# esa-prl/planning-motion_planning

Measured on AMD Instinct MI355X. Metric: Eikonal Gcells/s + ms-to-path, 4k² & 16k² costmap at 1/2/4/8 GPU, higher is better.
Workload: dtype f64; 1 GPU; C2: 4096x4096 DEM-derived cost raster, single goal, FIM on 1 MI355X; H=4096, W=4096, split=1x1, tile=64, parallelism=single-gpu

## Files before the change

planning-motion_planning_amd/csrc/fim2d.hip:

```cpp
#include "fim_engine.hpp"

namespace eik {

template <typename R>
__device__ __forceinline__ R stage_cost(R c) {
    if constexpr (sizeof(R) == 8 && EIK_CHAIN) return (c >= R(0) && c < 0x1p-500) ? R(0x1p-500) : c;
    else return c;
}


#ifndef EIK_ACT_STEP
#define EIK_ACT_STEP 0
#endif
constexpr int kActStep = EIK_ACT_STEP;



#ifndef EIK_ECOL_F64
#define EIK_ECOL_F64 1
#endif
#ifndef EIK_ECOL_F32
#define EIK_ECOL_F32 0
#endif
template <typename R>
constexpr bool kEcol = sizeof(R) == 8 ? EIK_ECOL_F64 : EIK_ECOL_F32;

#ifndef EIK_FRESH_SKIP
#define EIK_FRESH_SKIP 1
#endif
constexpr bool kFreshSkip = EIK_FRESH_SKIP;

template <typename R>
struct alignas(2 * sizeof(R)) Cell {
    R t, c;
};

#ifndef EIK_SWZ
#define EIK_SWZ 0
#endif
__device__ __forceinline__ constexpr int cell_swz(int col) { return EIK_SWZ ? (col >> 4) & 1 : 0; }
template <typename R>
__device__ __forceinline__ R& cell_t(Cell<R>* Ts, int idx, int col) {
    return reinterpret_cast<R*>(Ts + idx)[cell_swz(col)];
}
template <typename R>
__device__ __forceinline__ R& cell_c(Cell<R>* Ts, int idx, int col) {
    return reinterpret_cast<R*>(Ts + idx)[1 - cell_swz(col)];
}
template <typename R>
__device__ __forceinline__ Cell<R> make_cell(R t, R c, int col) {
    return cell_swz(col) ? Cell<R>{c, t} : Cell<R>{t, c};
}


#ifndef EIK_SWEEP_UNROLL
#define EIK_SWEEP_UNROLL 4
#endif
#ifndef EIK_SWEEP_UNROLL_F32
#define EIK_SWEEP_UNROLL_F32 8
#endif
template <typename R, int DX, int DY, bool TRACK, bool REF = false, class Hook>
__device__ __forceinline__ bool sweep_quadrant(Cell<R>* __restrict__ Ts, int lane, R keep, Hook&& hook) {
    constexpr int S = (int)sizeof(Cell<R>);
    constexpr int kRow = kLds * S;
    constexpr int D = kAhead;
    static_assert((2 * kTile) % D == 0, "pipeline depth must divide the step count");
    char* const base = reinterpret_cast<char*>(Ts);
    const int col = (DX > 0 ? lane : kTile - 1 - lane) + 1;
    constexpr int RB = (int)sizeof(R);
    const int colT = col * S + cell_swz(col) * RB;
    const int dC = (1 - 2 * cell_swz(col)) * RB;
    const int dU = (col - DX) * S + cell_swz(col - DX) * RB - colT;
    const int lo_b = -(D - 1) * kRow + colT, hi_b = (kLds - 1) * kRow + colT;
    int raw = DY > 0 ? (1 - lane) * kRow + colT : (kTile - (D - 1) + lane) * kRow + colT;
    auto off = [](int u) { return (DY > 0 ? u : D - 1 - u) * kRow; };
    auto clampb = [&](int x) {
        int r;
        asm("v_med3_i32 %0, %1, %2, %3" : "=v"(r) : "v"(x), "v"(lo_b), "v"(hi_b));
        return r;
    };
    bool changed = false;
    R cur = *reinterpret_cast<const R*>(base + (DY > 0 ? 0 : kLds - 1) * kRow + colT);
    R q_old[D], q_upx[D], q_c[D];
    int gb = clampb(raw);
    raw += DY * D * kRow;
    auto fetch = [&](int u) {
        const int o = gb + off(u);
#if EIK_SWZ
        q_old[u] = *reinterpret_cast<const R*>(base + o);
        q_c[u] = *reinterpret_cast<const R*>(base + o + dC);
#else
        const Cell<R> v = *reinterpret_cast<const Cell<R>*>(base + o);
        q_old[u] = v.t;
        q_c[u] = v.c;
#endif
        q_upx[u] = *reinterpret_cast<const R*>(base + o + dU);
    };
#pragma unroll
    for (int u = 0; u < D; ++u) fetch(u);
    constexpr int kUnroll = sizeof(R) == 8 ? EIK_SWEEP_UNROLL : EIK_SWEEP_UNROLL_F32;
#pragma unroll kUnroll
    for (int s = 0; s < 2 * kTile; s += D) {
        hook(s);
        const int gcur = gb;
        gb = clampb(raw);
        raw += DY * D * kRow;
#pragma unroll
        for (int u = 0; u < D; ++u) {
            const R c2x2 = R(2) * (q_c[u] * q_c[u]);
            R w;
            if constexpr (sizeof(R) == 8) {
                if constexpr (REF) w = eik_ref(wave_shr1(cur, q_upx[u]), cur, q_c[u]);
                else w = godunov2_chain(wave_shr1(cur, q_upx[u]), cur, q_c[u], c2x2);
                lds_min(reinterpret_cast<R*>(base + gcur + off(u)), w);
                if constexpr (TRACK) changed |= w < q_old[u] * keep;
                cur = fmin_nn(w, q_old[u]);
            } else {
                w = godunov2_chain(umin(wave_shr1_umin_id(cur), q_upx[u]), cur, q_c[u], c2x2);
                lds_min(reinterpret_cast<R*>(base + gcur + off(u)), w);
                if constexpr (TRACK) changed |= w < q_old[u] * keep;
                cur = umin(w, q_old[u]);
            }
            fetch(u);
            __builtin_amdgcn_sched_barrier(0);
        }
    }
    return changed;
}
template <typename R, int DX, int DY, bool TRACK, bool REF = false>
__device__ __forceinline__ bool sweep_quadrant(Cell<R>* __restrict__ Ts, int lane, R keep) {
    return sweep_quadrant<R, DX, DY, TRACK, REF>(Ts, lane, keep, [](int) {});
}

template <typename R>
struct TileLds {
    Cell<R> Tc[(kLds + 2 * kGuard) * kLds];
    unsigned round, flags;
    unsigned flags_acc;
    unsigned pend;
    unsigned key[5];
    int defer, tile, last;
    unsigned dirs;
    unsigned fresh;
};

template <typename R, bool COH, bool CAP = false, bool REF = false>
__device__ __forceinline__ void process_tile(const Fim2dArgs& a, int tile, TileLds<R>& L, R keep) {
    constexpr R INF = Real<R>::inf();
    Cell<R>* const Ts = L.Tc + kGuard * kLds;
    const int tid = threadIdx.x, lane = tid & 63, wave = tid >> 6;
    const int map = tile / a.tiles_per_map;
    const int rem = tile - map * a.tiles_per_map;
    const int ty = rem / a.ntx, tx = rem - (rem / a.ntx) * a.ntx;
    const R* __restrict__ cost = static_cast<const R*>(a.cost) + (int64_t)map * a.H * a.W;
    const TMem<R, COH> T(static_cast<R*>(a.T) + (int64_t)map * a.H * a.W, a.H * a.W);
    const TMem<R, COH> E(static_cast<R*>(a.ecol), (int64_t)a.capacity * 2 * kTile);
    auto eidx = [&](int t, int side, int row) { return ((int64_t)t * 2 + side) * kTile + row; };
    const int64_t y0 = (int64_t)ty * kTile, x0 = (int64_t)tx * kTile;
    const bool full = (y0 + kTile <= a.H) && (x0 + kTile <= a.W) && ((a.W & 3) == 0);
    const R capv = CAP ? (R)a.tcap[map] : INF;

    EIK_PROBE(0);
    if (tid == 0) {
        L.round = 0;
        L.flags = 0;
        L.flags_acc = 0;
        L.pend = 0;
    }
    if (tid < 5) L.key[tid] = 0x7f800000u;
    const int64_t sy = y0 + kTile < a.H ? y0 + kTile : a.H;
    const int64_t sx = x0 + kTile < a.W ? x0 + kTile : a.W;
    struct Halo {
        int h, hcol;
        int64_t hy, hx, idx;
        bool in;
    };
    auto halo_of = [&](int k) {
        Halo q;
        if (k == 0)      { q.hcol = lane + 1;            q.h = 0 * kLds + q.hcol; }
        else if (k == 1) { q.hcol = lane + 1;            q.h = (int)(sy - y0 + 1) * kLds + q.hcol; }
        else if (k == 2) { q.hcol = 0;                   q.h = (lane + 1) * kLds + q.hcol; }
        else             { q.hcol = (int)(sx - x0 + 1);  q.h = (lane + 1) * kLds + q.hcol; }
        q.hy = k == 0 ? y0 - 1 : k == 1 ? sy : y0 + lane;
        q.hx = k == 0 || k == 1 ? x0 + lane : k == 2 ? x0 - 1 : sx;
        q.in = q.hy >= 0 && q.hy < a.H && q.hx >= 0 && q.hx < a.W;
        q.idx = q.in ? q.hy * a.W + q.hx : 0;
        if (kEcol<R> && k >= 2 && q.in) q.idx = eidx(k == 2 ? tile - 1 : tile + 1, k == 2 ? 1 : 0, lane);
        return q;
    };
    auto load_halo_of = [&](const Halo& q, int k) {
        R v = kEcol<R> && k >= 2 ? E.ld(q.idx) : T.ld(q.idx);
        if (!q.in) v = load_T<R, COH>(a, T, q.hy, q.hx);
        return v;
    };
    const Halo hw = halo_of(wave);
    const int h = hw.h, hcol = hw.hcol;
    auto load_halo = [&]() { return load_halo_of(hw, wave); };
    R told[16];
    const int cx = (tid & 15) * 4;
    auto store_tile = [&](const R (&cr)[16], R hv) {
#pragma unroll
        for (int k = 0; k < 4; ++k) {
            const int ry = (tid >> 4) + 16 * k;
#pragma unroll
            for (int e = 0; e < 4; ++e)
                Ts[(ry + 1) * kLds + cx + e + 1] = make_cell<R>(told[4 * k + e], stage_cost(cr[4 * k + e]), cx + e + 1);
        }
        Ts[h] = make_cell<R>(hv, INF, hcol);
    };
    if (full && COH && kFreshSkip && __builtin_amdgcn_readfirstlane(L.fresh)) {
        R cr[16];
#pragma unroll
        for (int k = 0; k < 4; ++k) {
            const int64_t gy = y0 + (tid >> 4) + 16 * k;
            if constexpr (sizeof(R) == 4) {
                const float4 c4 = *reinterpret_cast<const float4*>(&cost[gy * a.W + x0 + cx]);
                cr[4 * k] = c4.x; cr[4 * k + 1] = c4.y; cr[4 * k + 2] = c4.z; cr[4 * k + 3] = c4.w;
            } else {
                const double2 c0 = *reinterpret_cast<const double2*>(&cost[gy * a.W + x0 + cx]);
                const double2 c1 = *reinterpret_cast<const double2*>(&cost[gy * a.W + x0 + cx + 2]);
                cr[4 * k] = c0.x; cr[4 * k + 1] = c0.y; cr[4 * k + 2] = c1.x; cr[4 * k + 3] = c1.y;
            }
#pragma unroll
            for (int e = 0; e < 4; ++e) told[4 * k + e] = INF;
        }
        store_tile(cr, load_halo());
        if (tid == 0) atomicAdd(a.visits + 2, 1ull);
    } else if (full) {
        R cr[16];
#pragma unroll
        for (int k = 0; k < 4; ++k) {
            const int64_t gy = y0 + (tid >> 4) + 16 * k;
            R tv[4];
            T.ld4(gy * a.W + x0 + cx, tv);
            if constexpr (sizeof(R) == 4) {
                const float4 c4 = *reinterpret_cast<const float4*>(&cost[gy * a.W + x0 + cx]);
                cr[4 * k] = c4.x; cr[4 * k + 1] = c4.y; cr[4 * k + 2] = c4.z; cr[4 * k + 3] = c4.w;
            } else {
                const double2 c0 = *reinterpret_cast<const double2*>(&cost[gy * a.W + x0 + cx]);
                const double2 c1 = *reinterpret_cast<const double2*>(&cost[gy * a.W + x0 + cx + 2]);
                cr[4 * k] = c0.x; cr[4 * k + 1] = c0.y; cr[4 * k + 2] = c1.x; cr[4 * k + 3] = c1.y;
            }
#pragma unroll
            for (int e = 0; e < 4; ++e) told[4 * k + e] = tv[e];
        }
        store_tile(cr, load_halo());
    } else {
        R cr[16];
#pragma unroll
        for (int k = 0; k < 4; ++k) {
            const int64_t gy = y0 + (tid >> 4) + 16 * k;
#pragma unroll
            for (int e = 0; e < 4; ++e) {
                const int64_t gx = x0 + cx + e;
                const bool in = gy < a.H && gx < a.W;
                told[4 * k + e] = load_T<R, COH>(a, T, gy, gx);
                cr[4 * k + e] = in ? cost[gy * a.W + gx] : INF;
            }
        }
        store_tile(cr, load_halo());
        if (tid < kLds) {
            if (sy - y0 < kTile) Ts[(kLds - 1) * kLds + tid] = Cell<R>{INF, INF};
            if (sx - x0 < kTile) Ts[tid * kLds + (kLds - 1)] = Cell<R>{INF, INF};
        }
    }
    if (lane < 4) cell_c(Ts, (lane >> 1) * (kLds - 1) * kLds + (lane & 1) * (kLds - 1), (lane & 1) * (kLds - 1)) = INF;
    __syncthreads();
    EIK_PROBE(1);
    if constexpr (CAP) asm volatile("" ::"v"(capv));

    unsigned dirs = L.dirs;
    int act_tile = -1;
    unsigned act_old = 0u, act_kold = 0x7f800000u;
    float act_k = 0.f;
    auto act_complete = [&]() {
        if (act_tile >= 0) qpush_complete(a, act_tile, act_old, act_k, act_kold);
        act_tile = -1;
    };
    for (int pass = 0;; ++pass) {
        auto hook = [&](int st) {
            if (EIK_ACT_SPLIT && wave == 0 && st == kActStep) act_complete();
        };
        const bool sweep = (dirs >> wave) & 1u;
        bool last_changed = false;
        if (a.max_rounds == 1) {
            if (sweep) {
                if (wave == 0)      sweep_quadrant<R, +1, +1, false, REF>(Ts, lane, keep, hook);
                else if (wave == 1) sweep_quadrant<R, -1, +1, false, REF>(Ts, lane, keep, hook);
                else if (wave == 2) sweep_quadrant<R, +1, -1, false, REF>(Ts, lane, keep, hook);
                else                sweep_quadrant<R, -1, -1, false, REF>(Ts, lane, keep, hook);
            } else {
                for (int st = 0; st < 2 * kTile; st += kAhead) hook(st);
            }
            __syncthreads();
        } else {
            for (int round = 0;; ++round) {
                bool ch = false;
                if (sweep) {
                    if (wave == 0)      ch = sweep_quadrant<R, +1, +1, true, REF>(Ts, lane, keep);
                    else if (wave == 1) ch = sweep_quadrant<R, -1, +1, true, REF>(Ts, lane, keep);
                    else if (wave == 2) ch = sweep_quadrant<R, +1, -1, true, REF>(Ts, lane, keep);
                    else                ch = sweep_quadrant<R, -1, -1, true, REF>(Ts, lane, keep);
                }
                if (__any(ch) && lane == 0) atomicOr(&L.round, 1u << (round & 31));
                __syncthreads();
                last_changed = (L.round >> (round & 31)) & 1u;
                if (!last_changed || round + 1 >= a.max_rounds) break;
            }
        }

        EIK_PROBE(2);
        unsigned pend_old = 0;
        R nv[16];
#pragma unroll
        for (int k = 0; k < 4; ++k) {
            const int ry = (tid >> 4) + 16 * k;
#pragma unroll
            for (int e = 0; e < 4; ++e) nv[4 * k + e] = cell_t(Ts, (ry + 1) * kLds + cx + e + 1, cx + e + 1);
        }
        unsigned chg = 0;
#pragma unroll
        for (int k = 0; k < 4; ++k) {
            const int ry = (tid >> 4) + 16 * k;
            const int64_t gy = y0 + ry;
            bool any = false;
#pragma unroll
            for (int e = 0; e < 4; ++e) {
                const int i = 4 * k + e;
                any |= nv[i] < told[i];
                const bool in = full || (gy < a.H && x0 + cx + e < a.W);
                chg |= (nv[i] < told[i] * keep && in) ? 1u << i : 0u;
            }
            if (any) {
                if (full) {
                    const R v[4] = {nv[4 * k], nv[4 * k + 1], nv[4 * k + 2], nv[4 * k + 3]};
                    T.st4(gy * a.W + x0 + cx, v);
                } else {
#pragma unroll
                    for (int e = 0; e < 4; ++e) {
                        const int64_t gx = x0 + cx + e;
                        if (gy < a.H && gx < a.W && nv[4 * k + e] < told[4 * k + e]) T.st(gy * a.W + gx, nv[4 * k + e]);
                    }
                }
                if (kEcol<R> && cx == 0 && nv[4 * k] < told[4 * k]) E.st(eidx(tile, 0, ry), nv[4 * k]);
                if (kEcol<R> && cx == kTile - 4 && nv[4 * k + 3] < told[4 * k + 3]) E.st(eidx(tile, 1, ry), nv[4 * k + 3]);
            }
        }
        if (COH && (a.sched & 1) && tid == 0)
            pend_old = atomicAnd(&a.qstate[tile + (int)__builtin_amdgcn_mbcnt_lo(0u, 0u)], kBusy | kVisited);
        __builtin_amdgcn_sched_barrier(0);
        if (COH) {
#pragma unroll
            for (int i = 0; i < 16; ++i) told[i] = nv[i];
        }
        const bool keys = a.delta < INF || a.bctl;
        unsigned fl = chg ? 128u : 0u;
        R kmin_self = INF, kmin[4] = {INF, INF, INF, INF};
        if (keys) {
#pragma unroll
            for (int i = 0; i < 16; ++i) kmin_self = umin(kmin_self, (chg >> i) & 1u ? nv[i] : INF);
        }
        auto edge = [&](int q, int i0, int di, int h0, int dh, int hc) {
            R hv[4];
#pragma unroll
            for (int j = 0; j < 4; ++j) hv[j] = cell_t(Ts, h0 + dh * j, hc < 0 ? cx + j + 1 : hc);
#pragma unroll
            for (int j = 0; j < 4; ++j) {
                const int i = i0 + di * j;
                const bool act = !CAP || nv[i] <= capv;
                const bool hit = ((chg >> i) & 1u) && act && nv[i] < hv[j];
                fl |= hit ? 1u << q : 0u;
                kmin[q] = umin(kmin[q], hit ? nv[i] : INF);
            }
        };
        const int ly0 = (tid >> 4) + 1;
        if ((tid >> 4) == 0) edge(0, 0, 1, cx + 1, 1, -1);
        if ((tid >> 4) == 15) edge(1, 12, 1, (kLds - 1) * kLds + cx + 1, 1, -1);
        if ((tid & 15) == 0) edge(2, 0, 4, ly0 * kLds, 16 * kLds, 0);
        if ((tid & 15) == 15) edge(3, 3, 4, ly0 * kLds + kLds - 1, 16 * kLds, kLds - 1);
        if (!full) {
#pragma unroll
            for (int k = 0; k < 4; ++k) {
                const int ry = (tid >> 4) + 16 * k;
                if (y0 + ry == a.H - 1 && ry != kTile - 1 && ((chg >> (4 * k)) & 0xFu)) fl |= 32u;
            }
#pragma unroll
            for (int e = 0; e < 4; ++e)
                if (x0 + cx + e == a.W - 1 && cx + e != kTile - 1 && (chg & (0x1111u << e))) fl |= 64u;
        }
        const unsigned wfl = wave_reduce_idem(fl, [](unsigned x, unsigned y) { return x | y; });
        if (wfl && lane == 0) atomicOr(&L.flags, wfl);
        if (keys) {
            const R km[5] = {kmin_self, kmin[0], kmin[1], kmin[2], kmin[3]};
#pragma unroll
            for (int q = 0; q < 5; ++q) {
                const unsigned wk = wave_reduce_idem(__float_as_uint((float)km[q]), [](unsigned x, unsigned y) { return min(x, y); });
                if (wk < 0x7f800000u && lane == 0) atomicMin(&L.key[q], wk);
            }
        }
        if (tid == 0) L.last = a.max_rounds == 1 ? -1 : (int)last_changed;
        if constexpr (COH) {
            __builtin_amdgcn_s_waitcnt(0x0F70);
            asm volatile("s_waitcnt vmcnt(0)" ::: "memory");
        }
        if (COH && (a.sched & 1) && tid == 0) L.pend = pend_old;
        __syncthreads();
        EIK_PROBE(7);
        if (COH) {
            const unsigned f = L.flags;
            const unsigned pend = L.pend & (kPending | kFromN | kFromS | kFromW | kFromE);
            const bool self = (f & 128u) != 0u;
            if ((!self && !pend) || pass + 1 >= a.max_passes || a.max_rounds != 1) break;
            const R hv = load_halo();
            if (tid == 64) charge_inplace_pass(a);
            const bool defer = (a.sched & 2) && pass > 0;
            if constexpr (EIK_ACT_SPLIT)
                act_tile = activate_neighbours_issue(a, tile, defer ? 0u : f, act_old, L.key, act_k,
                                                     act_kold);
            else
                activate_neighbours(a, tile, defer ? 0u : f, L.key, 0, 0u);
            if (defer && tid == 0) L.flags_acc |= f & 0x6fu;
            dirs = self ? 0xFu : sweep_dirs(pend);
            cell_t(Ts, h, hcol) = hv;
            __syncthreads();
            if (tid == 0) {
                L.flags = 0;
                L.pend = 0;
            }
        } else {
            break;
        }
    }
    act_complete();
    EIK_PROBE(3);
}

template <typename R>
__device__ __forceinline__ void activate_after(const Fim2dArgs& a, int tile, const TileLds<R>& L, int list,
                                               unsigned stamp) {
    const unsigned f = L.flags;
    activate_neighbours(a, tile, f | L.flags_acc, L.key, list, stamp);
    if (threadIdx.x == 0) {
        const bool self = L.last < 0 ? (f & 128u) != 0u : L.last != 0;
        if (a.mode == kModePersistent) {
            const unsigned p = L.pend & (kFromN | kFromS | kFromW | kFromE);
            if (self || (L.pend & kPending)) {
                if (self && a.bctl) atomicMin(&a.key[tile], 0u);
                atomicOr(&a.qstate[tile], kPending | (self ? kSelf : p));
            }
        } else if (self) {
            enqueue(a, tile, list, stamp, __uint_as_float(L.key[0]));
        }
    }
}

template <typename R>
__device__ __forceinline__ void init_guard_rows(TileLds<R>& L) {
    const int tid = threadIdx.x;
    for (int i = tid; i < kGuard * kLds; i += kThreads) {
        L.Tc[i] = Cell<R>{Real<R>::inf(), Real<R>::inf()};
        L.Tc[(kLds + kGuard) * kLds + i] = Cell<R>{Real<R>::inf(), Real<R>::inf()};
    }
}

template <typename R>
__global__ __launch_bounds__(kThreads) void fim2d_sweep_kernel(Fim2dArgs a) {
    constexpr R INF = Real<R>::inf();
    __shared__ TileLds<R> L;
    const int tid = threadIdx.x;
    init_guard_rows(L);
    const int cur = a.iter % 3, nxt = (a.iter + 1) % 3, rst = (a.iter + 2) % 3;
    const int cnt = a.counts[cur];
    if (blockIdx.x == 0 && tid == 0) {
        a.counts[rst] = 0;
        a.minkey[rst] = 0x7f800000u;
    }
    const unsigned stamp = a.iter + 2;
    const float thr = __uint_as_float(a.minkey[cur]) + a.delta;
    const R keep = (R)a.keep;
    if (tid == 0) L.dirs = 0xFu;

    for (int it = blockIdx.x; it < cnt; it += gridDim.x) {
        const int tile = a.lists[(int64_t)cur * a.capacity + it];
        if (a.delta < INF) {
            if (tid == 0) {
                const float k = __uint_as_float(atomicOr(&a.key[tile], 0u));
                L.defer = k > thr;
                if (k > thr) enqueue(a, tile, nxt, stamp, k);
                else atomicExch(&a.key[tile], 0x7f800000u);
            }
            __syncthreads();
            const bool defer = L.defer;
            __syncthreads();
            if (defer) continue;
        }
        process_tile<R, false>(a, tile, L, keep);
        activate_after(a, tile, L, nxt, stamp);
        if (tid == 0 && a.visits) atomicAdd(a.visits, 1ull);
        __syncthreads();
    }
}

template <typename R>
__device__ __forceinline__ void merge_strip_cells(const Fim2dArgs& a, int side, const R* rv, R* g, int64_t i,
                                                  int64_t len, unsigned* count) {
    R v = Real<R>::inf();
    bool drop = false;
    if (i < len) {
        v = ld_system(rv + i);
        drop = v < ld_agent(g + i);
        if (drop) st_scoped(g + i, v, __HIP_MEMORY_SCOPE_AGENT);
    }
    const unsigned long long m = __ballot(drop);
    if (!m) return;
    __builtin_amdgcn_fence(__ATOMIC_RELEASE, "agent");
    unsigned k = drop ? __float_as_uint((float)v) : 0x7f800000u;
#pragma unroll
    for (int d = 32; d > 0; d >>= 1) k = min(k, (unsigned)__shfl_xor((int)k, d));
    if ((threadIdx.x & 63) == (unsigned)__builtin_ctzll(m)) {
        if (count) atomicAdd(count, (unsigned)__popcll(m));
        int ty, tx;
        if (side < 2) {
            tx = (int)(i / kTile);
            ty = side == 0 ? 0 : a.nty - 1;
        } else {
            ty = (int)(i / kTile);
            tx = side == 2 ? 0 : a.ntx - 1;
        }
        activate(a, ty * a.ntx + tx, a.iter % 3, a.iter + 1, __uint_as_float(k), kFromN << side);
    }
}

template <typename R>
__device__ __forceinline__ void live_agent(const Fim2dArgs& a, unsigned* sh) {
    const int tid = threadIdx.x;
    auto pack = [&](unsigned par, bool skip_busy) {
        const R* T = static_cast<const R*>(a.T);
        R* tg[4];
        for (int k = 0; k < 4; ++k) tg[k] = static_cast<R*>(a.live->send[par][k]);
        auto idle = [&](int64_t ty, int64_t tx) {
            return !skip_busy ||
                   (__hip_atomic_load(&a.qstate[ty * a.ntx + tx], __ATOMIC_RELAXED, __HIP_MEMORY_SCOPE_AGENT) &
                    (kPending | kBusy)) == 0u;
        };
        for (int64_t i = tid; i < a.W; i += blockDim.x) {
            if (tg[0] && idle(0, i / kTile)) st_scoped(tg[0] + i, ld_agent(T + i), __HIP_MEMORY_SCOPE_SYSTEM);
            if (tg[1] && idle(a.nty - 1, i / kTile))
                st_scoped(tg[1] + i, ld_agent(T + (a.H - 1) * a.W + i), __HIP_MEMORY_SCOPE_SYSTEM);
        }
        for (int64_t i = tid; i < a.H; i += blockDim.x) {
            if (tg[2] && idle(i / kTile, 0)) st_scoped(tg[2] + i, ld_agent(T + i * a.W), __HIP_MEMORY_SCOPE_SYSTEM);
            if (tg[3] && idle(i / kTile, a.ntx - 1))
                st_scoped(tg[3] + i, ld_agent(T + i * a.W + a.W - 1), __HIP_MEMORY_SCOPE_SYSTEM);
        }
    };
    auto merge = [&](unsigned par, unsigned* count) {
        for (int side = 0; side < 4; ++side) {
            const R* rv = static_cast<const R*>(a.live->recv[par][side]);
            R* g = static_cast<R*>(const_cast<void*>(a.ghost[side]));
            if (!rv || !g) continue;
            const int64_t len = side < 2 ? a.W : a.H;
            for (int64_t i0 = 0; i0 < len; i0 += blockDim.x) merge_strip_cells<R>(a, side, rv, g, i0 + tid, len, count);
        }
    };
    live_agent_loop(a, sh, pack, merge);
}

template <typename R, int WPS, bool REF>
constexpr int kPersistWaves = WPS > 1 ? WPS : sizeof(R) == 4 ? 3 : REF ? 1 : 2;
template <typename R, int WPS, bool CAP = false, bool REF = false>
__global__ __launch_bounds__(kThreads, (kPersistWaves<R, WPS, REF>)) void fim2d_persist_kernel(Fim2dArgs a) {
    __shared__ TileLds<R> L;
    if (a.live && blockIdx.x == 0) {
        __shared__ unsigned sh[4];
        live_agent<R>(a, sh);
        return;
    }
    init_guard_rows(L);
    EIK_KSTART();
    const R keep = (R)a.keep;
    int tile = -1;
    unsigned nvis = 0;
    for (;;) {
        if (threadIdx.x < 64) {
            if (tile >= 0) {
                EIK_PROBE(4);
                activate_after(a, tile, L, 0, 0u);
                asm volatile("s_waitcnt vmcnt(0)" ::: "memory");
                if (threadIdx.x == 0) {
                    qfinish(a, tile);
                    if (++nvis == 64u) {
                        charge_visits(a, 64ull);
                        nvis = 0;
                    }
                }
            }
            EIK_PROBE(5);
        } else if (threadIdx.x < 128 && (a.bctl || threadIdx.x == 64)) {
            unsigned trig = 0;
            const int t = a.bctl ? qgrab_prio(a, trig) : qgrab(a, trig);
            if (threadIdx.x == 64) {
                L.tile = t;
                L.dirs = sweep_dirs(trig);
                L.fresh = !(trig & kVisited);
                if (t >= 0) EIK_VISIT(t, trig, L.dirs);
            }
        }
        __syncthreads();
        EIK_PROBE(6);
        tile = __builtin_amdgcn_readfirstlane(L.tile);
        if (tile < 0) break;
        process_tile<R, true, CAP, REF>(a, tile, L, keep);
    }
    if (threadIdx.x == 0 && nvis) atomicAdd(a.visits, (unsigned long long)nvis);
}
template <typename R>
__global__ void fim2d_init_kernel(R* __restrict__ T, int64_t n, unsigned* __restrict__ mark, int64_t ntiles,
                                  unsigned* __restrict__ key, unsigned* __restrict__ minkey, unsigned* __restrict__ qstate,
                                  unsigned* __restrict__ qslot, int64_t nslots, unsigned* __restrict__ counts,
                                  unsigned* __restrict__ qctl, unsigned* __restrict__ visits, unsigned* __restrict__ edge,
                                  R* __restrict__ ecol) {
    const int64_t stride = (int64_t)gridDim.x * blockDim.x;
    if (blockIdx.x == 0 && threadIdx.x < kQueueCtlBytes / 4) {
        const int t = threadIdx.x;
        if (qctl) qctl[t] = 0u;
        if (t < 4) {
            if (counts) counts[t] = 0u;
            if (edge) edge[t] = 0u;
        }
        if (t < 22 && visits) visits[t] = 0u;
    }
    for (int64_t i = (int64_t)blockIdx.x * blockDim.x + threadIdx.x; i < n; i += stride) T[i] = Real<R>::inf();
    if (ecol)
        for (int64_t i = (int64_t)blockIdx.x * blockDim.x + threadIdx.x; i < ntiles * 2 * kTile; i += stride)
            ecol[i] = Real<R>::inf();
    for (int64_t i = (int64_t)blockIdx.x * blockDim.x + threadIdx.x; i < ntiles; i += stride) {
        mark[i] = 0;
        key[i] = 0x7f800000u;
        if (qstate) qstate[i] = 0;
    }
    for (int64_t i = (int64_t)blockIdx.x * blockDim.x + threadIdx.x; i < nslots; i += stride) qslot[i] = 0;
    if (blockIdx.x == 0 && threadIdx.x < 3) minkey[threadIdx.x] = threadIdx.x == 0 ? 0u : 0x7f800000u;
}

template <typename R>
__global__ void fim2d_seed_kernel(Fim2dArgs a, const int64_t* __restrict__ goals, int nmaps) {
    const int m = blockIdx.x * blockDim.x + threadIdx.x;
    if (m == 0) {
        a.counts[1] = 0;
        a.counts[2] = 0;
    }
    if (m >= nmaps) return;
    const int64_t gx = goals[2 * m], gy = goals[2 * m + 1];
    if (gx < 0 || gy < 0 || gx >= a.W || gy >= a.H) return;
    static_cast<R*>(a.T)[(int64_t)m * a.H * a.W + gy * a.W + gx] = R(0);
    const int tile = m * a.tiles_per_map + (int)(gy / kTile) * a.ntx + (int)(gx / kTile);
    if (kEcol<R> && a.ecol && (gx % kTile == 0 || gx % kTile == kTile - 1))
        static_cast<R*>(a.ecol)[((int64_t)tile * 2 + (gx % kTile == 0 ? 0 : 1)) * kTile + gy % kTile] = R(0);
    if (a.mode == kModePersistent) {
        qpush(a, tile, kSelf | kVisited);
        return;
    }
    a.mark[tile] = 1;
    a.key[tile] = 0u;
    const int pos = atomicAdd(&a.counts[0], 1);
    a.lists[pos] = tile;
}

template <typename R>
__global__ __launch_bounds__(256) void prio_delta_kernel(const R* __restrict__ cost, int64_t n, float mult,
                                                          float* __restrict__ out) {
    __shared__ double ssum[4];
    __shared__ int scnt[4];
    double sum = 0.0;
    int cnt = 0;
    for (int i = threadIdx.x; i < 4096; i += 256) {
        const unsigned long long hsh = (unsigned long long)(i + 1) * 0x9E3779B97F4A7C15ull;
        const double c = (double)cost[(int64_t)((hsh >> 11) % (unsigned long long)n)];
        if (c > 0.0 && c < Real<double>::inf()) {
            sum += log(c);
            ++cnt;
        }
    }
    for (int d = 32; d > 0; d >>= 1) {
        sum += __shfl_down(sum, d);
        cnt += __shfl_down(cnt, d);
    }
    if ((threadIdx.x & 63) == 0) {
        ssum[threadIdx.x >> 6] = sum;
        scnt[threadIdx.x >> 6] = cnt;
    }
    __syncthreads();
    if (threadIdx.x == 0) {
        const double s = ssum[0] + ssum[1] + ssum[2] + ssum[3];
        const int c = scnt[0] + scnt[1] + scnt[2] + scnt[3];
        const double g = c ? exp(s / c) : 1.0;
        *out = (float)(mult * 64.0 * g > 1e-30 ? mult * 64.0 * g : 1e-30);
    }
}

hipError_t fim2d_prio_delta(const void* cost, bool f64, int64_t n, float mult, float* out, hipStream_t st) {
    if (f64)
        hipLaunchKernelGGL(prio_delta_kernel<double>, dim3(1), dim3(256), 0, st, static_cast<const double*>(cost), n,
                           mult, out);
    else
        hipLaunchKernelGGL(prio_delta_kernel<float>, dim3(1), dim3(256), 0, st, static_cast<const float*>(cost), n,
                           mult, out);
    return hipGetLastError();
}

__global__ void fim2d_qrewind_kernel(Fim2dArgs a) {
    if (a.bctl) {
        const int64_t stride = (int64_t)gridDim.x * blockDim.x;
        for (int64_t i = (int64_t)blockIdx.x * blockDim.x + threadIdx.x; i <= (int64_t)a.qmask; i += stride) {
            const unsigned v = a.qslot[i];
            if (v == 0u) continue;
            const unsigned tag = v >> kBandTagShift;
            if (tag) atomicAnd(&a.bmem[(v & kSlotTileMask) - 1u], ~(1ull << (tag - 1u)));
            a.qslot[i] = 0u;
        }
    }
    if (blockIdx.x == 0 && threadIdx.x == 0) *a.qhead = *a.qtail;
}
static void launch_qrewind(const Fim2dArgs& a, hipStream_t st) {
    const int grid = a.bctl ? (int)std::min<int64_t>(256, ((int64_t)a.qmask + 256) / 256) : 1;
    hipLaunchKernelGGL(fim2d_qrewind_kernel, dim3(grid), dim3(a.bctl ? 256 : 1), 0, st, a);
}

template <typename R>
__global__ __launch_bounds__(256) void fim2d_merge_ghost_kernel(Fim2dArgs a, int side, const R* __restrict__ recv,
                                                                int64_t len) {
    R* g = static_cast<R*>(const_cast<void*>(a.ghost[side]));
    merge_strip_cells<R>(a, side, recv, g, (int64_t)blockIdx.x * blockDim.x + threadIdx.x, len, nullptr);
}

template <typename R>
__global__ void fim2d_pack_edges_kernel(Fim2dArgs a, R* __restrict__ n, R* __restrict__ s, R* __restrict__ w,
                                        R* __restrict__ e) {
    const int64_t i = (int64_t)blockIdx.x * blockDim.x + threadIdx.x;
    const R* T = static_cast<const R*>(a.T);
    if (i < a.W) {
        if (n) st_scoped(n + i, ld_agent(T + i), __HIP_MEMORY_SCOPE_SYSTEM);
        if (s) st_scoped(s + i, ld_agent(T + (a.H - 1) * a.W + i), __HIP_MEMORY_SCOPE_SYSTEM);
    }
    if (i < a.H) {
        if (w) st_scoped(w + i, ld_agent(T + i * a.W), __HIP_MEMORY_SCOPE_SYSTEM);
        if (e) st_scoped(e + i, ld_agent(T + i * a.W + a.W - 1), __HIP_MEMORY_SCOPE_SYSTEM);
    }
}

hipError_t fim2d_sweep(const Fim2dArgs& a, bool f64, int grid, hipStream_t st) {
    if (f64)
        hipLaunchKernelGGL(fim2d_sweep_kernel<double>, dim3(grid), dim3(kThreads), 0, st, a);
    else
        hipLaunchKernelGGL(fim2d_sweep_kernel<float>, dim3(grid), dim3(kThreads), 0, st, a);
    return hipGetLastError();
}

int fim2d_persist_resident(bool f64, int cus, bool wide) {
    int per_cu = 0;
    const hipError_t e =
        f64    ? hipOccupancyMaxActiveBlocksPerMultiprocessor(&per_cu, fim2d_persist_kernel<double, 1>, kThreads, 0)
        : wide ? hipOccupancyMaxActiveBlocksPerMultiprocessor(&per_cu, fim2d_persist_kernel<float, 4>, kThreads, 0)
               : hipOccupancyMaxActiveBlocksPerMultiprocessor(&per_cu, fim2d_persist_kernel<float, 1>, kThreads, 0);
    if (e != hipSuccess || per_cu < 1) per_cu = 1;
    return per_cu * cus;
}

hipError_t fim2d_persist(const Fim2dArgs& a, bool f64, int grid, hipStream_t st, bool wide, bool rewind) {
    if (f64 && a.ref_arith && a.tcap)
        hipLaunchKernelGGL((fim2d_persist_kernel<double, 1, true, true>), dim3(grid), dim3(kThreads), 0, st, a);
    else if (f64 && a.ref_arith)
        hipLaunchKernelGGL((fim2d_persist_kernel<double, 1, false, true>), dim3(grid), dim3(kThreads), 0, st, a);
    else if (f64 && a.tcap)
        hipLaunchKernelGGL((fim2d_persist_kernel<double, 1, true>), dim3(grid), dim3(kThreads), 0, st, a);
    else if (f64)
        hipLaunchKernelGGL((fim2d_persist_kernel<double, 1>), dim3(grid), dim3(kThreads), 0, st, a);
    else if (wide)
        hipLaunchKernelGGL((fim2d_persist_kernel<float, 4>), dim3(grid), dim3(kThreads), 0, st, a);
    else
        hipLaunchKernelGGL((fim2d_persist_kernel<float, 1>), dim3(grid), dim3(kThreads), 0, st, a);
    if (rewind) launch_qrewind(a, st);
    return hipGetLastError();
}

hipError_t fim2d_qrewind(const Fim2dArgs& a, hipStream_t st) {
    launch_qrewind(a, st);
    return hipGetLastError();
}

hipError_t fim2d_init(const Fim2dArgs& a, bool f64, int nmaps, const int64_t* d_goals, unsigned* edge, hipStream_t st) {
    static_assert(kQueueCtlBytes / 4 <= 256, "the init kernel's block 0 clears the queue words");
    const int64_t n = (int64_t)nmaps * a.H * a.W;
    const int64_t ntiles = (int64_t)nmaps * a.tiles_per_map;
    const int grid = (int)std::min<int64_t>(4096, (n + 255) / 256);
    const int64_t nslots = a.qslot ? (int64_t)a.qmask + 1 : 0;
    unsigned* const counts = reinterpret_cast<unsigned*>(a.counts);
    unsigned* const qctl = reinterpret_cast<unsigned*>(a.qhead);
    unsigned* const visits = reinterpret_cast<unsigned*>(a.visits);
    if (f64) {
        hipLaunchKernelGGL(fim2d_init_kernel<double>, dim3(grid), dim3(256), 0, st, static_cast<double*>(a.T), n,
                           a.mark, ntiles, a.key, a.minkey, a.qstate, a.qslot, nslots, counts, qctl, visits, edge,
                           kEcol<double> ? static_cast<double*>(a.ecol) : nullptr);
        hipLaunchKernelGGL(fim2d_seed_kernel<double>, dim3((nmaps + 255) / 256), dim3(256), 0, st, a, d_goals, nmaps);
    } else {
        hipLaunchKernelGGL(fim2d_init_kernel<float>, dim3(grid), dim3(256), 0, st, static_cast<float*>(a.T), n,
                           a.mark, ntiles, a.key, a.minkey, a.qstate, a.qslot, nslots, counts, qctl, visits, edge,
                           kEcol<float> ? static_cast<float*>(a.ecol) : nullptr);
        hipLaunchKernelGGL(fim2d_seed_kernel<float>, dim3((nmaps + 255) / 256), dim3(256), 0, st, a, d_goals, nmaps);
    }
    return hipGetLastError();
}

hipError_t fim2d_merge_ghost(const Fim2dArgs& a, bool f64, int side, const void* recv, int64_t len, hipStream_t st) {
    const int grid = (int)((len + 255) / 256);
    if (f64)
        hipLaunchKernelGGL(fim2d_merge_ghost_kernel<double>, dim3(grid), dim3(256), 0, st, a, side,
                           static_cast<const double*>(recv), len);
    else
        hipLaunchKernelGGL(fim2d_merge_ghost_kernel<float>, dim3(grid), dim3(256), 0, st, a, side,
                           static_cast<const float*>(recv), len);
    return hipGetLastError();
}

hipError_t fim2d_pack_edges(const Fim2dArgs& a, bool f64, void* n, void* s, void* w, void* e, hipStream_t st) {
    const int64_t len = a.H > a.W ? a.H : a.W;
    const int grid = (int)((len + 255) / 256);
    if (f64)
        hipLaunchKernelGGL(fim2d_pack_edges_kernel<double>, dim3(grid), dim3(256), 0, st, a, (double*)n, (double*)s,
                           (double*)w, (double*)e);
    else
        hipLaunchKernelGGL(fim2d_pack_edges_kernel<float>, dim3(grid), dim3(256), 0, st, a, (float*)n, (float*)s,
                           (float*)w, (float*)e);
    return hipGetLastError();
}

}
```

Before: 8.599 Gcells/s.

## Precompute halo source pointers, pin tile geometry in SGPRs, clamp edge-tile loads

Tile geometry is passed in a struct pinned to scalar registers, and the wave index is made uniform. Halo loads on full tiles now take a per-wave base pointer and stride chosen branchlessly, including ghost buffers, instead of recomputing per-lane bounds logic. Partial-edge f64 tiles use clamped unconditional loads followed by masking, and store predicates reuse a precomputed in-bounds mask. The seed kernel also activates neighbouring tiles when the goal sits on a tile edge, which changes scheduling slightly and adds complexity and some risk in the ghost and edge handling.

```diff
diff --git a/planning-motion_planning_amd/csrc/fim2d.hip b/planning-motion_planning_amd/csrc/fim2d.hip
--- a/planning-motion_planning_amd/csrc/fim2d.hip
+++ b/planning-motion_planning_amd/csrc/fim2d.hip
@@ -29,6 +29,9 @@
 #define EIK_FRESH_SKIP 1
 #endif
 constexpr bool kFreshSkip = EIK_FRESH_SKIP;
+
+template <typename R>
+constexpr bool kCutWide = sizeof(R) == 8;
 
 template <typename R>
 struct alignas(2 * sizeof(R)) Cell {
@@ -144,20 +147,25 @@
     unsigned fresh;
 };
 
+struct TileGeom {
+    int64_t H, W;
+    int ntx, tiles_per_map, max_passes;
+};
 template <typename R, bool COH, bool CAP = false, bool REF = false>
-__device__ __forceinline__ void process_tile(const Fim2dArgs& a, int tile, TileLds<R>& L, R keep) {
+__device__ __forceinline__ void process_tile(const Fim2dArgs& a, const TileGeom& g, int tile, TileLds<R>& L, R keep) {
     constexpr R INF = Real<R>::inf();
     Cell<R>* const Ts = L.Tc + kGuard * kLds;
-    const int tid = threadIdx.x, lane = tid & 63, wave = tid >> 6;
-    const int map = tile / a.tiles_per_map;
-    const int rem = tile - map * a.tiles_per_map;
-    const int ty = rem / a.ntx, tx = rem - (rem / a.ntx) * a.ntx;
-    const R* __restrict__ cost = static_cast<const R*>(a.cost) + (int64_t)map * a.H * a.W;
-    const TMem<R, COH> T(static_cast<R*>(a.T) + (int64_t)map * a.H * a.W, a.H * a.W);
+    const int tid = threadIdx.x, lane = tid & 63;
+    const int wave = __builtin_amdgcn_readfirstlane(tid >> 6);
+    const int map = tile / g.tiles_per_map;
+    const int rem = tile - map * g.tiles_per_map;
+    const int ty = rem / g.ntx, tx = rem - (rem / g.ntx) * g.ntx;
+    const R* __restrict__ cost = static_cast<const R*>(a.cost) + (int64_t)map * g.H * g.W;
+    const TMem<R, COH> T(static_cast<R*>(a.T) + (int64_t)map * g.H * g.W, g.H * g.W);
     const TMem<R, COH> E(static_cast<R*>(a.ecol), (int64_t)a.capacity * 2 * kTile);
     auto eidx = [&](int t, int side, int row) { return ((int64_t)t * 2 + side) * kTile + row; };
     const int64_t y0 = (int64_t)ty * kTile, x0 = (int64_t)tx * kTile;
-    const bool full = (y0 + kTile <= a.H) && (x0 + kTile <= a.W) && ((a.W & 3) == 0);
+    const bool full = (y0 + kTile <= g.H) && (x0 + kTile <= g.W) && ((g.W & 3) == 0);
     const R capv = CAP ? (R)a.tcap[map] : INF;
 
     EIK_PROBE(0);
@@ -168,8 +176,8 @@
         L.pend = 0;
     }
     if (tid < 5) L.key[tid] = 0x7f800000u;
-    const int64_t sy = y0 + kTile < a.H ? y0 + kTile : a.H;
-    const int64_t sx = x0 + kTile < a.W ? x0 + kTile : a.W;
+    const int64_t sy = y0 + kTile < g.H ? y0 + kTile : g.H;
+    const int64_t sx = x0 + kTile < g.W ? x0 + kTile : g.W;
     struct Halo {
         int h, hcol;
         int64_t hy, hx, idx;
@@ -183,22 +191,55 @@
         else             { q.hcol = (int)(sx - x0 + 1);  q.h = (lane + 1) * kLds + q.hcol; }
         q.hy = k == 0 ? y0 - 1 : k == 1 ? sy : y0 + lane;
         q.hx = k == 0 || k == 1 ? x0 + lane : k == 2 ? x0 - 1 : sx;
-        q.in = q.hy >= 0 && q.hy < a.H && q.hx >= 0 && q.hx < a.W;
-        q.idx = q.in ? q.hy * a.W + q.hx : 0;
+        q.in = q.hy >= 0 && q.hy < g.H && q.hx >= 0 && q.hx < g.W;
+        q.idx = q.in ? q.hy * g.W + q.hx : 0;
         if (kEcol<R> && k >= 2 && q.in) q.idx = eidx(k == 2 ? tile - 1 : tile + 1, k == 2 ? 1 : 0, lane);
         return q;
     };
-    auto load_halo_of = [&](const Halo& q, int k) {
+    const bool ghosts = a.ghost[0] || a.ghost[1] || a.ghost[2] || a.ghost[3];
+    auto load_halo_of = [&](int k) {
+        const Halo q = halo_of(k);
         R v = kEcol<R> && k >= 2 ? E.ld(q.idx) : T.ld(q.idx);
-        if (!q.in) v = load_T<R, COH>(a, T, q.hy, q.hx);
+        if (ghosts) {
+            if (!q.in) v = load_T<R, COH>(a, T, q.hy, q.hx);
+        } else {
+            v = q.in ? v : INF;
+        }
         return v;
     };
-    const Halo hw = halo_of(wave);
-    const int h = hw.h, hcol = hw.hcol;
-    auto load_halo = [&]() { return load_halo_of(hw, wave); };
+    const int hcol = wave < 2 ? lane + 1 : wave == 2 ? 0 : (int)(sx - x0 + 1);
+    const int h = (wave == 0 ? 0 : wave == 1 ? (int)(sy - y0 + 1) : lane + 1) * kLds + hcol;
+    TMem<R, COH> HM = T;
+    int hidx = 0;
+    bool hsrc = true;
+    auto halo_source = [&]() {
+        if constexpr (COH) {
+            const bool row = wave < 2;
+            const bool in = wave == 0 ? y0 > 0 : wave == 1 ? sy < g.H : wave == 2 ? x0 > 0 : sx < g.W;
+            auto gbits = [&](int k) { return reinterpret_cast<uintptr_t>(a.ghost[k]) & (uintptr_t)0 - (uintptr_t)(wave == k); };
+            R* const gs = reinterpret_cast<R*>(gbits(0) | gbits(1) | gbits(2) | gbits(3));
+            R* const Tm = static_cast<R*>(a.T) + (int64_t)map * g.H * g.W;
+            const bool ecol = kEcol<R> && !row;
+            R* const base = !in ? gs : ecol ? static_cast<R*>(a.ecol) : Tm;
+            const int64_t n = !in ? (gs ? (row ? g.W : g.H) : 0) : ecol ? (int64_t)a.capacity * 2 * kTile : (int64_t)g.H * g.W;
+            const int64_t first = !in    ? (row ? x0 : y0)
+                                  : row  ? (wave == 0 ? y0 - 1 : sy) * g.W + x0
+                                  : ecol ? eidx(wave == 2 ? tile - 1 : tile + 1, wave == 2 ? 1 : 0, 0)
+                                         : y0 * g.W + (wave == 2 ? x0 - 1 : sx);
+            const int64_t stride = in && !row && !ecol ? g.W : 1;
+            HM = TMem<R, COH>(base, n);
+            hidx = (int)(first + lane * stride);
+            hsrc = in || gs;
+        }
+    };
+    auto halo_issue_full = [&]() -> R {
+        if constexpr (COH) return HM.ld(hidx);
+        else return load_halo_of(wave);
+    };
     R told[16];
+    unsigned inm = 0xFFFFu;
     const int cx = (tid & 15) * 4;
-    auto store_tile = [&](const R (&cr)[16], R hv) {
+    auto store_tile = [&](const R (&cr)[16], R hv, bool src) {
 #pragma unroll
         for (int k = 0; k < 4; ++k) {
             const int ry = (tid >> 4) + 16 * k;
@@ -206,7 +247,8 @@
             for (int e = 0; e < 4; ++e)
                 Ts[(ry + 1) * kLds + cx + e + 1] = make_cell<R>(told[4 * k + e], stage_cost(cr[4 * k + e]), cx + e + 1);
         }
-        Ts[h] = make_cell<R>(hv, INF, hcol);
+        if (src) Ts[h] = make_cell<R>(hv, INF, hcol);
+        else Ts[h] = make_cell<R>(INF, INF, hcol);
     };
     if (full && COH && kFreshSkip && __builtin_amdgcn_readfirstlane(L.fresh)) {
         R cr[16];
@@ -214,17 +256,20 @@
         for (int k = 0; k < 4; ++k) {
             const int64_t gy = y0 + (tid >> 4) + 16 * k;
             if constexpr (sizeof(R) == 4) {
-                const float4 c4 = *reinterpret_cast<const float4*>(&cost[gy * a.W + x0 + cx]);
+                const float4 c4 = *reinterpret_cast<const float4*>(&cost[gy * g.W + x0 + cx]);
                 cr[4 * k] = c4.x; cr[4 * k + 1] = c4.y; cr[4 * k + 2] = c4.z; cr[4 * k + 3] = c4.w;
             } else {
-                const double2 c0 = *reinterpret_cast<const double2*>(&cost[gy * a.W + x0 + cx]);
-                const double2 c1 = *reinterpret_cast<const double2*>(&cost[gy * a.W + x0 + cx + 2]);
+                const double2 c0 = *reinterpret_cast<const double2*>(&cost[gy * g.W + x0 + cx]);
+                const double2 c1 = *reinterpret_cast<const double2*>(&cost[gy * g.W + x0 + cx + 2]);
                 cr[4 * k] = c0.x; cr[4 * k + 1] = c0.y; cr[4 * k + 2] = c1.x; cr[4 * k + 3] = c1.y;
             }
 #pragma unroll
             for (int e = 0; e < 4; ++e) told[4 * k + e] = INF;
         }
-        store_tile(cr, load_halo());
+        halo_source();
+        const R hraw = halo_issue_full();
+        __builtin_amdgcn_sched_barrier(0);
+        store_tile(cr, hraw, !COH || hsrc);
         if (tid == 0) atomicAdd(a.visits + 2, 1ull);
     } else if (full) {
         R cr[16];
@@ -232,33 +277,63 @@
         for (int k = 0; k < 4; ++k) {
             const int64_t gy = y0 + (tid >> 4) + 16 * k;
             R tv[4];
-            T.ld4(gy * a.W + x0 + cx, tv);
+            T.ld4(gy * g.W + x0 + cx, tv);
             if constexpr (sizeof(R) == 4) {
-                const float4 c4 = *reinterpret_cast<const float4*>(&cost[gy * a.W + x0 + cx]);
+                const float4 c4 = *reinterpret_cast<const float4*>(&cost[gy * g.W + x0 + cx]);
                 cr[4 * k] = c4.x; cr[4 * k + 1] = c4.y; cr[4 * k + 2] = c4.z; cr[4 * k + 3] = c4.w;
             } else {
-                const double2 c0 = *reinterpret_cast<const double2*>(&cost[gy * a.W + x0 + cx]);
-                const double2 c1 = *reinterpret_cast<const double2*>(&cost[gy * a.W + x0 + cx + 2]);
+                const double2 c0 = *reinterpret_cast<const double2*>(&cost[gy * g.W + x0 + cx]);
+                const double2 c1 = *reinterpret_cast<const double2*>(&cost[gy * g.W + x0 + cx + 2]);
                 cr[4 * k] = c0.x; cr[4 * k + 1] = c0.y; cr[4 * k + 2] = c1.x; cr[4 * k + 3] = c1.y;
             }
 #pragma unroll
             for (int e = 0; e < 4; ++e) told[4 * k + e] = tv[e];
         }
-        store_tile(cr, load_halo());
+        halo_source();
+        const R hraw = halo_issue_full();
+        __builtin_amdgcn_sched_barrier(0);
+        store_tile(cr, hraw, !COH || hsrc);
     } else {
         R cr[16];
+        inm = 0u;
+        const int rmax = (int)(g.H - 1 - y0), cmax = (int)(g.W - 1 - x0);
+        const int64_t org = y0 * g.W + x0;
 #pragma unroll
         for (int k = 0; k < 4; ++k) {
-            const int64_t gy = y0 + (tid >> 4) + 16 * k;
+            const int ry = (tid >> 4) + 16 * k;
+            const int row = (ry < rmax ? ry : rmax) * (int)g.W;
 #pragma unroll
             for (int e = 0; e < 4; ++e) {
-                const int64_t gx = x0 + cx + e;
-                const bool in = gy < a.H && gx < a.W;
-                told[4 * k + e] = load_T<R, COH>(a, T, gy, gx);
-                cr[4 * k + e] = in ? cost[gy * a.W + gx] : INF;
-            }
-        }
-        store_tile(cr, load_halo());
+                const bool in = ry <= rmax && cx + e <= cmax;
+                const int64_t idx = org + (row + (cx + e < cmax ? cx + e : cmax));
+                inm |= in ? 1u << (4 * k + e) : 0u;
+                if constexpr (kCutWide<R>) {
+                    told[4 * k + e] = T.ld(idx);
+                    cr[4 * k + e] = cost[idx];
+                } else {
+                    told[4 * k + e] = load_T<R, COH>(a, T, y0 + ry, x0 + cx + e);
+                    cr[4 * k + e] = in ? cost[(y0 + ry) * g.W + x0 + cx + e] : INF;
+                }
+            }
+        }
+        const R hv = load_halo_of(wave);
+        if constexpr (kCutWide<R>) {
+            if (ghosts) {
+#pragma unroll
+                for (int k = 0; k < 4; ++k) {
+                    const int64_t gy = y0 + (tid >> 4) + 16 * k;
+#pragma unroll
+                    for (int e = 0; e < 4; ++e)
+                        if (!((inm >> (4 * k + e)) & 1u)) told[4 * k + e] = load_T<R, COH>(a, T, gy, x0 + cx + e);
+                }
+            } else {
+#pragma unroll
+                for (int i = 0; i < 16; ++i) told[i] = (inm >> i) & 1u ? told[i] : INF;
+            }
+#pragma unroll
+            for (int i = 0; i < 16; ++i) cr[i] = (inm >> i) & 1u ? cr[i] : INF;
+        }
+        store_tile(cr, hv, true);
         if (tid < kLds) {
             if (sy - y0 < kTile) Ts[(kLds - 1) * kLds + tid] = Cell<R>{INF, INF};
             if (sx - x0 < kTile) Ts[tid * kLds + (kLds - 1)] = Cell<R>{INF, INF};
@@ -319,6 +394,8 @@
             for (int e = 0; e < 4; ++e) nv[4 * k + e] = cell_t(Ts, (ry + 1) * kLds + cx + e + 1, cx + e + 1);
         }
         unsigned chg = 0;
+        unsigned inp = inm;
+        asm volatile("" : "+v"(inp));
 #pragma unroll
         for (int k = 0; k < 4; ++k) {
             const int ry = (tid >> 4) + 16 * k;
@@ -328,24 +405,24 @@
             for (int e = 0; e < 4; ++e) {
                 const int i = 4 * k + e;
                 any |= nv[i] < told[i];
-                const bool in = full || (gy < a.H && x0 + cx + e < a.W);
-                chg |= (nv[i] < told[i] * keep && in) ? 1u << i : 0u;
+                chg |= nv[i] < told[i] * keep ? 1u << i : 0u;
             }
             if (any) {
                 if (full) {
                     const R v[4] = {nv[4 * k], nv[4 * k + 1], nv[4 * k + 2], nv[4 * k + 3]};
-                    T.st4(gy * a.W + x0 + cx, v);
+                    T.st4(gy * g.W + x0 + cx, v);
                 } else {
 #pragma unroll
                     for (int e = 0; e < 4; ++e) {
                         const int64_t gx = x0 + cx + e;
-                        if (gy < a.H && gx < a.W && nv[4 * k + e] < told[4 * k + e]) T.st(gy * a.W + gx, nv[4 * k + e]);
+                        if (((inp >> (4 * k + e)) & 1u) && nv[4 * k + e] < told[4 * k + e]) T.st(gy * g.W + gx, nv[4 * k + e]);
                     }
                 }
                 if (kEcol<R> && cx == 0 && nv[4 * k] < told[4 * k]) E.st(eidx(tile, 0, ry), nv[4 * k]);
                 if (kEcol<R> && cx == kTile - 4 && nv[4 * k + 3] < told[4 * k + 3]) E.st(eidx(tile, 1, ry), nv[4 * k + 3]);
             }
         }
+        chg &= inp;
         if (COH && (a.sched & 1) && tid == 0)
             pend_old = atomicAnd(&a.qstate[tile + (int)__builtin_amdgcn_mbcnt_lo(0u, 0u)], kBusy | kVisited);
         __builtin_amdgcn_sched_barrier(0);
@@ -382,11 +459,11 @@
 #pragma unroll
             for (int k = 0; k < 4; ++k) {
                 const int ry = (tid >> 4) + 16 * k;
-                if (y0 + ry == a.H - 1 && ry != kTile - 1 && ((chg >> (4 * k)) & 0xFu)) fl |= 32u;
+                if (y0 + ry == g.H - 1 && ry != kTile - 1 && ((chg >> (4 * k)) & 0xFu)) fl |= 32u;
             }
 #pragma unroll
             for (int e = 0; e < 4; ++e)
-                if (x0 + cx + e == a.W - 1 && cx + e != kTile - 1 && (chg & (0x1111u << e))) fl |= 64u;
+                if (x0 + cx + e == g.W - 1 && cx + e != kTile - 1 && (chg & (0x1111u << e))) fl |= 64u;
         }
         const unsigned wfl = wave_reduce_idem(fl, [](unsigned x, unsigned y) { return x | y; });
         if (wfl && lane == 0) atomicOr(&L.flags, wfl);
@@ -410,8 +487,11 @@
             const unsigned f = L.flags;
             const unsigned pend = L.pend & (kPending | kFromN | kFromS | kFromW | kFromE);
             const bool self = (f & 128u) != 0u;
-            if ((!self && !pend) || pass + 1 >= a.max_passes || a.max_rounds != 1) break;
-            const R hv = load_halo();
+            if ((!self && !pend) || pass + 1 >= g.max_passes || a.max_rounds != 1) break;
+            const bool hfast = COH && full;
+            R hv;
+            if (hfast) hv = halo_issue_full();
+            else hv = load_halo_of(wave);
             if (tid == 64) charge_inplace_pass(a);
             const bool defer = (a.sched & 2) && pass > 0;
             if constexpr (EIK_ACT_SPLIT)
@@ -421,7 +501,7 @@
                 activate_neighbours(a, tile, defer ? 0u : f, L.key, 0, 0u);
             if (defer && tid == 0) L.flags_acc |= f & 0x6fu;
             dirs = self ? 0xFu : sweep_dirs(pend);
-            cell_t(Ts, h, hcol) = hv;
+            if (!hfast || hsrc) cell_t(Ts, h, hcol) = hv;
             __syncthreads();
             if (tid == 0) {
                 L.flags = 0;
@@ -479,6 +559,7 @@
     const float thr = __uint_as_float(a.minkey[cur]) + a.delta;
     const R keep = (R)a.keep;
     if (tid == 0) L.dirs = 0xFu;
+    const TileGeom g{a.H, a.W, a.ntx, a.tiles_per_map, a.max_passes};
 
     for (int it = blockIdx.x; it < cnt; it += gridDim.x) {
         const int tile = a.lists[(int64_t)cur * a.capacity + it];
@@ -494,7 +575,7 @@
             __syncthreads();
             if (defer) continue;
         }
-        process_tile<R, false>(a, tile, L, keep);
+        process_tile<R, false>(a, g, tile, L, keep);
         activate_after(a, tile, L, nxt, stamp);
         if (tid == 0 && a.visits) atomicAdd(a.visits, 1ull);
         __syncthreads();
@@ -579,6 +660,8 @@
     init_guard_rows(L);
     EIK_KSTART();
     const R keep = (R)a.keep;
+    TileGeom g{a.H, a.W, a.ntx, a.tiles_per_map, a.max_passes};
+    asm volatile("" : "+s"(g.H), "+s"(g.W), "+s"(g.ntx), "+s"(g.tiles_per_map), "+s"(g.max_passes));
     int tile = -1;
     unsigned nvis = 0;
     for (;;) {
@@ -610,7 +693,7 @@
         EIK_PROBE(6);
         tile = __builtin_amdgcn_readfirstlane(L.tile);
         if (tile < 0) break;
-        process_tile<R, true, CAP, REF>(a, tile, L, keep);
+        process_tile<R, true, CAP, REF>(a, g, tile, L, keep);
     }
     if (threadIdx.x == 0 && nvis) atomicAdd(a.visits, (unsigned long long)nvis);
 }
@@ -659,12 +742,17 @@
         static_cast<R*>(a.ecol)[((int64_t)tile * 2 + (gx % kTile == 0 ? 0 : 1)) * kTile + gy % kTile] = R(0);
     if (a.mode == kModePersistent) {
         qpush(a, tile, kSelf | kVisited);
-        return;
-    }
-    a.mark[tile] = 1;
-    a.key[tile] = 0u;
-    const int pos = atomicAdd(&a.counts[0], 1);
-    a.lists[pos] = tile;
+    } else {
+        a.mark[tile] = 1;
+        a.key[tile] = 0u;
+        const int pos = atomicAdd(&a.counts[0], 1);
+        a.lists[pos] = tile;
+    }
+    const int ty = (int)(gy / kTile), tx = (int)(gx / kTile);
+    if (gy % kTile == 0 && ty > 0) activate(a, tile - a.ntx, 0, 1u, 0.f, kFromS);
+    if (gy % kTile == kTile - 1 && ty + 1 < a.nty) activate(a, tile + a.ntx, 0, 1u, 0.f, kFromN);
+    if (gx % kTile == 0 && tx > 0) activate(a, tile - 1, 0, 1u, 0.f, kFromE);
+    if (gx % kTile == kTile - 1 && tx + 1 < a.ntx) activate(a, tile + 1, 0, 1u, 0.f, kFromW);
 }
 
 template <typename R>
```

Measured after the change: 8.655 Gcells/s (median of 6 runs). About the same (+0.7%).
